# RoyiAvital/QuadraticProgramSolver

Hardware: AMD Instinct MI355X
Metric: ADMM iterations/sec (higher is better)
Workload: dtype f64

## Files before the change

quadraticprogramsolver_amd/csrc/k_loop.hip:

```cpp
#include <cstdlib>

#include "qps_kernels.h"
#include "wave_reduce.h"
#include <hip/hip_ext.h>

namespace qps {

namespace {

template <typename T> __device__ __forceinline__ T wave_sum(T v) { return wave_sum_all(v); }
__device__ __forceinline__ unsigned long long absbits(double v) { return (unsigned long long)__double_as_longlong(fabs(v)); }
__device__ __forceinline__ unsigned long long wave_max_u64(unsigned long long v) {
#pragma unroll
    for (int o = 32; o > 0; o >>= 1) { unsigned long long t = __shfl_xor(v, o, 64); v = t > v ? t : v; }
    return v;
}

template <typename T, int RB, int TRI, int THREADS>
__global__ __launch_bounds__(THREADS) void k_gemv_rows(const T* __restrict__ S, int64_t ld, const T* __restrict__ v,
                                                   T* __restrict__ out, const T* __restrict__ out0, T alpha, T beta,
                                                   int r0, int c0, int c1, BatchStride bs) {
    using V = typename VecOf<T>::type;
    if (bs.active && !bs.active[blockIdx.y]) return;
    S += (int64_t)blockIdx.y * bs.mat; v += (int64_t)blockIdx.y * bs.vin; out += (int64_t)blockIdx.y * bs.vout;
    if (out0) out0 += (int64_t)blockIdx.y * bs.vout;
    constexpr int VN = VecOf<T>::N;
    constexpr int CHUNK = THREADS * VN;
    const int tid = threadIdx.x;
    const int rb = r0 + (TRI == 1 ? (int)(gridDim.x - 1 - blockIdx.x) : (int)blockIdx.x) * RB;
    int cb = c0, ce = c1;
    if (TRI == 1) ce = min(c1, rb + RB);
    if (TRI == 2) cb = max(c0, rb);
    T acc[RB];
#pragma unroll
    for (int i = 0; i < RB; ++i) acc[i] = T(0);
    const T* Srow = S + (int64_t)rb * ld;
#pragma unroll 4
    for (int c = cb + tid * VN; c < ce; c += CHUNK) {
        const V vv = *reinterpret_cast<const V*>(v + c);
        const T* vp = reinterpret_cast<const T*>(&vv);
#pragma unroll
        for (int i = 0; i < RB; ++i) {
            typedef T NV __attribute__((ext_vector_type(VN)));
            const NV* src = reinterpret_cast<const NV*>(Srow + (int64_t)i * ld + c);
            const NV a = (TRI == 0) ? __builtin_nontemporal_load(src) : *src;
            T ap[VN];
#pragma unroll
            for (int e = 0; e < VN; ++e) ap[e] = a[e];
#pragma unroll
            for (int e = 0; e < VN; ++e) {
                bool ok = true;
                if (TRI == 1) ok = (c + e) <= (rb + i);
                if (TRI == 2) ok = (c + e) >= (rb + i);
                acc[i] += ok ? ap[e] * vp[e] : T(0);
            }
        }
    }
    __shared__ T red[THREADS / 64][RB];
#pragma unroll
    for (int i = 0; i < RB; ++i) acc[i] = wave_sum(acc[i]);
    if ((tid & 63) == 0) {
#pragma unroll
        for (int i = 0; i < RB; ++i) red[tid >> 6][i] = acc[i];
    }
    __syncthreads();
    if (tid < RB) {
        T s = T(0);
#pragma unroll
        for (int w = 0; w < THREADS / 64; ++w) s += red[w][tid];
        T r = alpha * s;
        if (beta != T(0)) r += beta * out0[rb + tid];
        out[rb + tid] = r;
    }
}

constexpr int GC_RT = 32;
template <typename T>
__global__ __launch_bounds__(256) void k_gemv_cols(const T* __restrict__ S, int64_t ld, const T* __restrict__ va,
                                                   const T* __restrict__ vb, T ca, T cb, T* __restrict__ part,
                                                   int64_t part_ld, int ncols) {
    using V = typename VecOf<T>::type;
    constexpr int VN = VecOf<T>::N;
    const int c = (blockIdx.x * 256 + threadIdx.x) * VN;
    if (c >= ncols) return;
    const int rt = blockIdx.y;
    const int rbase = rt * GC_RT;
    T acc[VN];
#pragma unroll
    for (int e = 0; e < VN; ++e) acc[e] = T(0);
    const T* Sp = S + (int64_t)rbase * ld + c;
#pragma unroll 8
    for (int i = 0; i < GC_RT; ++i) {
        T w = ca * va[rbase + i];
        if (vb) w += cb * vb[rbase + i];
        typedef T NV __attribute__((ext_vector_type(VN)));
        const NV a = __builtin_nontemporal_load(reinterpret_cast<const NV*>(Sp + (int64_t)i * ld));
#pragma unroll
        for (int e = 0; e < VN; ++e) acc[e] += a[e] * w;
    }
    V o;
    T* op = reinterpret_cast<T*>(&o);
#pragma unroll
    for (int e = 0; e < VN; ++e) op[e] = acc[e];
    *reinterpret_cast<V*>(part + (int64_t)rt * part_ld + c) = o;
}

template <typename T>
__global__ __launch_bounds__(256) void k_colsum(const T* __restrict__ part, int64_t part_ld, int ntiles,
                                                const T* __restrict__ a0, T s0, const T* __restrict__ a1, T s1,
                                                T* __restrict__ out, int ncols, BatchStride bs) {
    using V = typename VecOf<T>::type;
    constexpr int VN = VecOf<T>::N;
    if (bs.active && !bs.active[blockIdx.y]) return;
    part += (int64_t)blockIdx.y * bs.mat; out += (int64_t)blockIdx.y * bs.vout;
    if (a0) a0 += (int64_t)blockIdx.y * bs.vin;
    if (a1) a1 += (int64_t)blockIdx.y * bs.vin;
    constexpr int COLS = 128 / (int)sizeof(T);
    constexpr int CL = COLS / VN;
    constexpr int TL = 256 / CL;
    const int cl = threadIdx.x % CL, tl = threadIdx.x / CL;
    const int c = blockIdx.x * COLS + cl * VN;
    T acc[VN];
#pragma unroll
    for (int e = 0; e < VN; ++e) acc[e] = T(0);
    if (c < ncols) {
        int t = tl;
        for (; t + 7 * TL < ntiles; t += 8 * TL) {
            V v[8];
#pragma unroll
            for (int j = 0; j < 8; ++j) v[j] = *reinterpret_cast<const V*>(part + (int64_t)(t + TL * j) * part_ld + c);
#pragma unroll
            for (int j = 0; j < 8; ++j) {
                const T* vp = reinterpret_cast<const T*>(&v[j]);
#pragma unroll
                for (int e = 0; e < VN; ++e) acc[e] += vp[e];
            }
        }
        for (; t < ntiles; t += TL) {
            const V v = *reinterpret_cast<const V*>(part + (int64_t)t * part_ld + c);
            const T* vp = reinterpret_cast<const T*>(&v);
#pragma unroll
            for (int e = 0; e < VN; ++e) acc[e] += vp[e];
        }
    }
    __shared__ T red[TL][COLS + 1];
#pragma unroll
    for (int e = 0; e < VN; ++e) red[tl][cl * VN + e] = acc[e];
    __syncthreads();
    constexpr int PL = 256 / COLS;
    static_assert(TL % PL == 0 && (PL == 16 || PL == 8), "slab lanes per output");
    const int o = threadIdx.x / PL, pl = threadIdx.x % PL;
    T s = T(0);
#pragma unroll
    for (int k = 0; k < TL / PL; ++k) s += red[pl * (TL / PL) + k][o];
    s = (PL == 16) ? row16_sum_last(s) : oct_sum_all(s);
    const int oc = blockIdx.x * COLS + o;
    if (pl == PL - 1 && oc < ncols) {
        T r = s;
        if (a0) r += s0 * a0[oc];
        if (a1) r += s1 * a1[oc];
        out[oc] = r;
    }
}

template <typename T>
__global__ __launch_bounds__(256) void k_admm_update(int NP, int MP, const T* __restrict__ xx, const T* __restrict__ zz,
                                                     T* __restrict__ x, T* __restrict__ xp, T* __restrict__ z,
                                                     T* __restrict__ zp, T* __restrict__ y, const T* __restrict__ l,
                                                     const T* __restrict__ u, T alpha, T rho) {
    const int i = blockIdx.x * 256 + threadIdx.x;
    const T alpha1 = T(1) - alpha, rho1 = T(1) / rho;
    if (i < NP) {
        const T xo = x[i];
        xp[i] = xo;
        x[i] = alpha * xx[i] + alpha1 * xo;
    }
    if (i < MP) {
        const T zo = z[i], yo = y[i], zt = zz[i];
        zp[i] = zo;
        T t = alpha * zt + alpha1 * zo + rho1 * yo;
        const T lo = l[i], hi = u[i];
        const T zn = t > hi ? hi : (t < lo ? lo : t);
        z[i] = zn;
        y[i] = yo + rho * (alpha * zt + alpha1 * zo - zn);
    }
}

template <typename T>
__global__ __launch_bounds__(256) void k_check_norms(int n, int m, const T* __restrict__ Ax, const T* __restrict__ Px,
                                                     const T* __restrict__ Aty, const T* __restrict__ q,
                                                     const T* __restrict__ x, const T* __restrict__ xp,
                                                     const T* __restrict__ z, const T* __restrict__ zp,
                                                     unsigned long long* __restrict__ slots, int dual_only, BatchStride bs) {
    if (bs.active && !bs.active[blockIdx.y]) return;
    {
        const int64_t on = (int64_t)blockIdx.y * bs.vin, om = (int64_t)blockIdx.y * bs.vout;
        Ax += om; z += om; zp += om; Px += on; Aty += on; q += on; x += on; xp += on; slots += (int64_t)blockIdx.y * 16;
    }
    unsigned long long v[9];
#pragma unroll
    for (int k = 0; k < 9; ++k) v[k] = 0ull;
    for (int i = blockIdx.x * 256 + threadIdx.x; i < max(n, m); i += gridDim.x * 256) {
        if (i < m && !dual_only) {
            const double ax = (double)Ax[i], zi = (double)z[i];
            v[0] = max(v[0], absbits((double)(Ax[i] - z[i])));
            v[2] = max(v[2], absbits(ax));
            v[3] = max(v[3], absbits(zi));
            v[8] = max(v[8], absbits((double)(z[i] - zp[i])));
        }
        if (i < n) {
            v[1] = max(v[1], absbits((double)(Px[i] + q[i] + Aty[i])));
            v[4] = max(v[4], absbits((double)Px[i]));
            v[5] = max(v[5], absbits((double)Aty[i]));
            v[6] = max(v[6], absbits((double)q[i]));
            if (!dual_only) v[7] = max(v[7], absbits((double)(x[i] - xp[i])));
        }
    }
#pragma unroll
    for (int k = 0; k < 9; ++k) {
        v[k] = wave_max_u64(v[k]);
        if ((threadIdx.x & 63) == 0 && v[k] != 0ull) atomicMax(&slots[k], v[k]);
    }
}

__device__ __forceinline__ double jmax(double a, double b) { return (isnan(a) || isnan(b)) ? (double)NAN : (a > b ? a : b); }

__global__ void k_check_decide(const unsigned long long* __restrict__ slots, double* __restrict__ res, CheckScalars cs,
                               const double* __restrict__ rho_arr, const double* __restrict__ rhorho_arr,
                               const int* __restrict__ active) {
    if (threadIdx.x != 0) return;
    const int b = blockIdx.x;
    if (active && !active[b]) return;
    slots += (int64_t)b * 16; res += (int64_t)b * 8;
    if (rho_arr) { cs.rho = rho_arr[b]; cs.rhorho = rhorho_arr[b]; cs.convFlag = 1; }
    double nv[9];
    for (int k = 0; k < 9; ++k) nv[k] = __longlong_as_double((long long)slots[k]);
    const double MIN_VAL_RHO = 1e-3, MAX_VAL_RHO = 1e6;
    const double normResPrim = nv[0], normResDual = nv[1];
    const double maxNormPrim = jmax(nv[2], nv[3]);
    const double maxNormDual = jmax(jmax(nv[4], nv[5]), nv[6]);
    double rhorho = cs.rhorho;
    if (cs.adptRho) {
        const double numeratorVal = normResPrim * maxNormDual;
        const double denominatorVal = normResDual * maxNormPrim;
        const double t = cs.rho * sqrt(numeratorVal / denominatorVal);
        rhorho = t > MAX_VAL_RHO ? MAX_VAL_RHO : (t < MIN_VAL_RHO ? MIN_VAL_RHO : t);
    }
    const double epsPrim = cs.epsAbs + cs.epsRel * maxNormPrim;
    const double epsDual = cs.epsAbs + cs.epsRel * maxNormDual;
    int flag = cs.convFlag;
    if ((normResPrim < epsPrim) && (normResDual < epsDual)) flag = 3;
    if ((nv[7] <= cs.epsAdmm) && (nv[8] <= cs.epsAdmm)) flag = 2;
    res[0] = normResPrim; res[1] = normResDual; res[2] = maxNormPrim; res[3] = maxNormDual;
    res[4] = rhorho; res[5] = (double)flag; res[6] = nv[7]; res[7] = nv[8];
}

template <typename T> __global__ void k_fill(T* p, int64_t n, T v) {
    int64_t i = (int64_t)blockIdx.x * 256 + threadIdx.x;
    if (i < n) p[i] = v;
}
template <typename T> __global__ void k_convert(const double* __restrict__ s, T* __restrict__ d, int64_t n) {
    int64_t i = (int64_t)blockIdx.x * 256 + threadIdx.x;
    if (i < n) d[i] = (T)s[i];
}
template <typename T> __global__ void k_convert_back(const T* __restrict__ s, double* __restrict__ d, int64_t n) {
    int64_t i = (int64_t)blockIdx.x * 256 + threadIdx.x;
    if (i < n) d[i] = (double)s[i];
}

}

static int env_int(const char* name, int dflt) { const char* e = getenv(name); return e ? atoi(e) : dflt; }

template <typename T, int RB, int TH>
static void gemv_rows_launch(hipStream_t st, const T* S, int64_t ld, const T* v, T* out, const T* out0, T alpha, T beta, int r0,
                             int r1, int c0, int c1, int tri, BatchStride bs) {
    dim3 grid((r1 - r0 + RB - 1) / RB, bs.count);
#define QPS_GR(TRI) hipLaunchKernelGGL((k_gemv_rows<T, RB, TRI, TH>), grid, dim3(TH), 0, st, S, ld, v, out, out0, alpha, beta, r0, c0, c1, bs)
    if (tri == 0) QPS_GR(0); else if (tri == 1) QPS_GR(1); else QPS_GR(2);
#undef QPS_GR
}

template <typename T>
void gemv_rows(hipStream_t st, const T* S, int64_t ld, const T* v, T* out, const T* out0, T alpha, T beta, int r0, int r1,
               int c0, int c1, int tri, BatchStride bs) {
    if (r1 <= r0) return;
    static const int wide_th = env_int("QPS_GEMV_WIDE_THREADS", 512);
    static const int wide_rb = env_int("QPS_GEMV_WIDE_RB", 2);
    const bool wide = (c1 - c0) >= 4 * 256 * VecOf<T>::N;
    if (!wide) { gemv_rows_launch<T, 4, 256>(st, S, ld, v, out, out0, alpha, beta, r0, r1, c0, c1, tri, bs); return; }
#define QPS_W(RB, TH) gemv_rows_launch<T, RB, TH>(st, S, ld, v, out, out0, alpha, beta, r0, r1, c0, c1, tri, bs)
    if (wide_th == 512) { if (wide_rb == 4) QPS_W(4, 512); else QPS_W(VecOf<T>::N == 2 ? 2 : 4, 512); }
    else if (wide_th == 256) { if (wide_rb == 4) QPS_W(4, 256); else QPS_W(VecOf<T>::N == 2 ? 2 : 4, 256); }
    else { if (wide_rb == 4) QPS_W(4, 1024); else QPS_W(VecOf<T>::N == 2 ? 2 : 4, 1024); }
#undef QPS_W
}

int gemv_cols_tiles(int nrows) { return (nrows + GC_RT - 1) / GC_RT; }

template <typename T>
int gemv_cols_partial(hipStream_t st, const T* S, int64_t ld, const T* va, const T* vb, T ca, T cb, T* part,
                      int64_t part_ld, int nrows, int ncols) {
    constexpr int VN = VecOf<T>::N;
    const int tiles = gemv_cols_tiles(nrows);
    if (tiles == 0) return 0;
    dim3 grid((ncols + 256 * VN - 1) / (256 * VN), tiles), block(256);
    hipLaunchKernelGGL((k_gemv_cols<T>), grid, block, 0, st, S, ld, va, vb, ca, cb, part, part_ld, ncols);
    return tiles;
}

template <typename T>
void colsum(hipStream_t st, const T* part, int64_t part_ld, int ntiles, const T* a0, T s0, const T* a1, T s1, T* out,
            int ncols, BatchStride bs) {
    constexpr int cols_wg = 128 / (int)sizeof(T);
    if (g_launch_timing.start) {
        const LaunchTiming lt = g_launch_timing;
        g_launch_timing = LaunchTiming();
        hipExtLaunchKernelGGL((k_colsum<T>), dim3((ncols + cols_wg - 1) / cols_wg, bs.count), dim3(256), 0, st, lt.start, lt.stop, 0, part, part_ld, ntiles, a0, s0, a1, s1, out, ncols, bs);
        return;
    }
    hipLaunchKernelGGL((k_colsum<T>), dim3((ncols + cols_wg - 1) / cols_wg, bs.count), dim3(256), 0, st, part, part_ld, ntiles, a0, s0, a1, s1, out, ncols, bs);
}

template <typename T>
void admm_update(hipStream_t st, int NP, int MP, const T* xx, const T* zz, T* x, T* xp, T* z, T* zp, T* y, const T* l,
                 const T* u, T alpha, T rho) {
    const int N = NP > MP ? NP : MP;
    hipLaunchKernelGGL((k_admm_update<T>), dim3((N + 255) / 256), dim3(256), 0, st, NP, MP, xx, zz, x, xp, z, zp, y, l, u, alpha, rho);
}

template <typename T>
void check_convergence(hipStream_t st, int n, int m, const T* Ax, const T* Px, const T* Aty, const T* q, const T* x,
                       const T* xp, const T* z, const T* zp, unsigned long long* scratch, double* res_dev, CheckScalars cs,
                       int dual_only, BatchStride bs, const double* rho_arr, const double* rhorho_arr) {
    if (!dual_only) (void)hipMemsetAsync(scratch, 0, 16 * sizeof(unsigned long long) * bs.count, st);
    const int N = n > m ? n : m;
    int blocks = (N + 255) / 256;
    if (blocks > 1024) blocks = 1024;
    if (blocks < 1) blocks = 1;
    hipLaunchKernelGGL((k_check_norms<T>), dim3(blocks, bs.count), dim3(256), 0, st, n, m, Ax, Px, Aty, q, x, xp, z, zp, scratch, dual_only, bs);
    hipLaunchKernelGGL(k_check_decide, dim3(bs.count), dim3(64), 0, st, scratch, res_dev, cs, rho_arr, rhorho_arr, bs.active);
}

template <typename T> void fill(hipStream_t st, T* p, int64_t n, T v) {
    if (n <= 0) return;
    hipLaunchKernelGGL((k_fill<T>), dim3((unsigned)((n + 255) / 256)), dim3(256), 0, st, p, n, v);
}
template <typename T> void convert_copy(hipStream_t st, const double* src, T* dst, int64_t n) {
    if (n <= 0) return;
    hipLaunchKernelGGL((k_convert<T>), dim3((unsigned)((n + 255) / 256)), dim3(256), 0, st, src, dst, n);
}
template <typename T> void convert_back(hipStream_t st, const T* src, double* dst, int64_t n) {
    if (n <= 0) return;
    hipLaunchKernelGGL((k_convert_back<T>), dim3((unsigned)((n + 255) / 256)), dim3(256), 0, st, src, dst, n);
}

#define INST(T)                                                                                                              \
    template void gemv_rows<T>(hipStream_t, const T*, int64_t, const T*, T*, const T*, T, T, int, int, int, int, int, BatchStride); \
    template int gemv_cols_partial<T>(hipStream_t, const T*, int64_t, const T*, const T*, T, T, T*, int64_t, int, int);      \
    template void colsum<T>(hipStream_t, const T*, int64_t, int, const T*, T, const T*, T, T*, int, BatchStride);            \
    template void admm_update<T>(hipStream_t, int, int, const T*, const T*, T*, T*, T*, T*, T*, const T*, const T*, T, T);   \
    template void check_convergence<T>(hipStream_t, int, int, const T*, const T*, const T*, const T*, const T*, const T*,    \
                                       const T*, const T*, unsigned long long*, double*, CheckScalars, int, BatchStride,     \
                                       const double*, const double*);                                                        \
    template void fill<T>(hipStream_t, T*, int64_t, T);                                                                      \
    template void convert_copy<T>(hipStream_t, const double*, T*, int64_t);                                                  \
    template void convert_back<T>(hipStream_t, const T*, double*, int64_t);
INST(double)
INST(float)
#undef INST

}
```

quadraticprogramsolver_amd/csrc/qps_dense_batch.hip:

```cpp
#include <memory>

#include "dense_chol.h"
#include "qps_batch.h"
#include "qps_internal.h"
#include "qps_kernels.h"
#include "qps_polish.h"

namespace qps {
namespace {

template <typename T> struct BatchedDenseSolver : BatchSolverBase {
    StreamLease lease; DeviceOwner mem; hipStream_t st = nullptr;
    int NP = 0, MP = 0, nb = 0, slabs = 0, rpw = 0, part_tiles = 0;
    T *A = nullptr, *P = nullptr, *q = nullptr, *l = nullptr, *u = nullptr, *PI = nullptr, *AA = nullptr, *M = nullptr, *S = nullptr,
      *tmp = nullptr, *dinv = nullptr;
    T *x = nullptr, *xp = nullptr, *xres = nullptr, *z = nullptr, *y = nullptr, *xx = nullptr, *tt = nullptr, *yv = nullptr, *part = nullptr,
      *part2 = nullptr, *part_tmp = nullptr, *sw_part = nullptr, *Px = nullptr, *Aty = nullptr;
    int* fail = nullptr; int* d_active = nullptr; double *d_rho = nullptr, *d_rhorho = nullptr;
    unsigned long long* scratch = nullptr; double* res_dev = nullptr; double* res_host = nullptr; double* stage = nullptr;
    int* h_int = nullptr; double* h_dbl = nullptr;
    bool have_AA = false; double fac_sigma = -1; int fac_nb = -1; std::vector<double> fac_rho;
    char* sb_args = nullptr; void* sb_host = nullptr;
    int cat_pass = 0, cat_sweep = 0;
    static constexpr const char* kWhat = "P + sigma I + rho A'A";

    BatchedDenseSolver(int dev, int cnt, int64_t n_, int64_t m_) {
        device = dev; n = n_; m = m_; count = cnt;
        HIPC(hipSetDevice(device));
        st = prof.st = lease.acquire(device);
        NP = roundup(n, 64); MP = roundup(m, 64);
        slabs = apass_plan<T>(NP, MP, &rpw, count);
        {
            const double s = sizeof(T), c = cnt;
            cat_pass = prof.category("apass(fused A-pass, batched)", c * s * ((double)m * n + 3.0 * n + 6.0 * m));
            cat_sweep = prof.category("sweeps(fused fwd+bwd, batched, triangle read once)", c * s * ((double)n * (n + 1) / 2 + 2.0 * n));
        }
        part_tiles = gemv_cols_tiles(MP);
        const int64_t nn = (int64_t)NP * NP, c = count;
        A = mem.dalloc<T>(c * MP * NP, st); P = mem.dalloc<T>(c * nn, st); PI = mem.dalloc<T>(c * nn, st); AA = mem.dalloc<T>(c * nn, st); M = mem.dalloc<T>(c * nn, st);
        S = mem.dalloc<T>(c * nn, st); tmp = mem.dalloc<T>(c * nn, st); dinv = mem.dalloc<T>(c * (int64_t)(NP / 64) * 4096, st);
        q = mem.dalloc<T>(c * NP, st); l = mem.dalloc<T>(c * MP, st); u = mem.dalloc<T>(c * MP, st);
        x = mem.dalloc<T>(c * NP, st); xp = mem.dalloc<T>(c * NP, st); xres = mem.dalloc<T>(c * NP, st); xx = mem.dalloc<T>(c * NP, st); tt = mem.dalloc<T>(c * NP, st);
        yv = mem.dalloc<T>(c * NP, st); Px = mem.dalloc<T>(c * NP, st); Aty = mem.dalloc<T>(c * NP, st); z = mem.dalloc<T>(c * MP, st); y = mem.dalloc<T>(c * MP, st);
        int rpw1 = 0;
        const int64_t part_slabs = std::max<int64_t>(std::max<int64_t>(c * slabs, apass_plan<T>(NP, MP, &rpw1, 1)), std::max(part_tiles, 1));
        part = mem.dalloc<T>(part_slabs * NP, st); part2 = mem.dalloc<T>(c * slabs * NP, st); part_tmp = mem.dalloc<T>((int64_t)std::max(part_tiles, 1) * NP, st);
        const int sw_slabs = sweep_fused_slabs<T>(NP, count); sw_part = mem.dalloc<T>(c * std::max(sw_slabs, 1) * NP, st);
        fail = mem.dalloc<int>(count + 4, st); d_active = mem.dalloc<int>(count + 4, st); d_rho = mem.dalloc<double>(count + 4, st); d_rhorho = mem.dalloc<double>(count + 4, st);
        scratch = mem.dalloc<unsigned long long>(16 * c, st); res_dev = mem.dalloc<double>(8 * c, st);
        res_host = mem.pinned<double>(8 * c); h_int = mem.pinned<int>(count + 4); h_dbl = mem.pinned<double>(2 * (count + 4));
        stage = mem.dalloc<double>(std::max<int64_t>((int64_t)MP * NP, nn) + 64, st);
    }
    ~BatchedDenseSolver() override {
        (void)hipSetDevice(device);
        (void)hipStreamSynchronize(st);
        prof.release_events();
    }
    std::unique_ptr<FastUploader> loader;
    void put_vec(const double* h, T* d, int64_t cnt_) {
        if (cnt_ <= 0) return;
        if (!loader) loader.reset(new FastUploader(st, device));
        loader->copy(stage, h, sizeof(double) * (size_t)cnt_);
        convert_copy<T>(st, stage, d, cnt_);
    }
    void put_matrix(const double* h, int rows, int cols, T* d) {
        if (rows <= 0 || cols <= 0) return;
        if (!loader) loader.reset(new FastUploader(st, device));
        loader->copy(stage, h, sizeof(double) * (size_t)rows * cols);
        import_colmajor<T>(st, stage, rows, rows, cols, d, NP);
    }
    void finish_loading() { HIPC(hipStreamSynchronize(st)); loader.reset(); }
    void get_dual(double* zh, double* yh) override {
        HIPC(hipSetDevice(device));
        for (int b = 0; b < count && m > 0; ++b) {
            if (zh) HIPC(download_staged<T>(st, stage, z + (int64_t)b * MP, zh + (int64_t)b * m, m));
            if (yh) HIPC(download_staged<T>(st, stage, y + (int64_t)b * MP, yh + (int64_t)b * m, m));
        }
    }
    void load_problem(int b, const double* Ph, const double* Ah, const double* qh, const double* lh, const double* uh) {
        put_matrix(Ph, (int)n, (int)n, P + (int64_t)b * NP * NP);
        put_matrix(Ah, (int)m, (int)n, A + (int64_t)b * MP * NP);
        put_vec(qh, q + (int64_t)b * NP, n); put_vec(lh, l + (int64_t)b * MP, m); put_vec(uh, u + (int64_t)b * MP, m);
    }
    DenseChol<T> chol() const { return {st, (int)n, NP, MP, P, A, PI, AA, M, S, tmp, dinv, fail}; }
    void push_state(const std::vector<double>& rho, const std::vector<double>& rhorho, const std::vector<int>& active) {
        for (int b = 0; b < count; ++b) { h_dbl[b] = rho[b]; h_dbl[count + 4 + b] = rhorho[b]; h_int[b] = active[b]; }
        HIPC(hipMemcpyAsync(d_rho, h_dbl, sizeof(double) * count, hipMemcpyHostToDevice, st));
        HIPC(hipMemcpyAsync(d_rhorho, h_dbl + count + 4, sizeof(double) * count, hipMemcpyHostToDevice, st));
        HIPC(hipMemcpyAsync(d_active, h_int, sizeof(int) * count, hipMemcpyHostToDevice, st));
        HIPC(hipStreamSynchronize(st));
    }

    void refactor_changed(const std::vector<int>& changed, double sigma, const std::vector<double>& rho, const std::vector<double>& rhorho,
                          const std::vector<int>& active, std::vector<double>& tref, bool rebuild_slabs, bool push_after) {
        const double ta = now_s();
        const DenseChol<T> ch = chol();
        const bool together = (int)changed.size() * 2 >= count;
        if (together) {
            push_state(rho, rhorho, active);
            ch.form(sigma, 0.0, false, false, count, d_rho);
            ch.factor(nb, count);
            for (int b = 0; b < count; ++b) fac_rho[b] = rho[b];
        }
        for (int b : changed) {
            if (!together) { ch.at(b).form(sigma, rho[b], false, false); ch.at(b).factor(nb); fac_rho[b] = rho[b]; }
            if (rebuild_slabs) {
                T* pb_ = part + (int64_t)b * slabs * NP;
                gemv_cols_partial<T>(st, A + (int64_t)b * MP * NP, NP, z + (int64_t)b * MP, y + (int64_t)b * MP, (T)rho[b], T(-1), part_tmp, NP, MP, NP);
                colsum<T>(st, part_tmp, NP, part_tiles, nullptr, T(0), nullptr, T(0), pb_, NP);
                if (slabs > 1) HIPC(hipMemsetAsync(pb_ + NP, 0, sizeof(T) * (size_t)(slabs - 1) * NP, st));
            }
        }
        std::vector<int> all(count);
        for (int b = 0; b < count; ++b) all[b] = b;
        ch.check(kWhat, "", h_int, count, together ? &all : &changed);
        if (push_after) push_state(rho, rhorho, active);
        const double dt = (now_s() - ta) / changed.size();
        for (int b : changed) tref[b] += dt;
    }

    void solve_batch(double* xh, const qps_params& p, qps_info* infos) override {
        HIPC(hipSetDevice(device));
        const double t0 = now_s();
        if (slabs <= 0) throw QpsError(QPS_ERR_UNSUPPORTED, "batched path needs m >= 1 and n within the fused-pass limit");
        nb = pick_nb<T>(p.trsvBlock, NP);
        const DenseChol<T> ch = chol();
        const double sigma = p.sigma, alpha = p.alpha;
        const double epsAdmm = std::fmin(p.epsAbs, p.epsRel) * 1e-2;
        std::vector<double> rho(count, p.rho), rhorho(count, p.rho), resP(count, NAN), resD(count, NAN), tref(count, 0.0);
        std::vector<int> active(count, 1), conv(count, QPS_CONV_NUM_ITR), iters(count, p.numIterations), nref(count, 0);
        HIPC(hipMemsetAsync(fail, 0, sizeof(int) * count, st));
        const bool rebuild = !(p.reuseFactor && have_AA && fac_sigma == sigma);
        if ((int)fac_rho.size() != count) fac_rho.assign(count, -1.0);
        std::vector<int> todo;
        for (int b = 0; b < count; ++b)
            if (rebuild || fac_rho[b] != p.rho || fac_nb != nb) todo.push_back(b);
        if ((int)todo.size() == count) { ch.form(sigma, p.rho, rebuild, rebuild, count); ch.factor(nb, count); }
        else for (int b : todo) { ch.at(b).form(sigma, p.rho, rebuild, rebuild); ch.at(b).factor(nb); }
        ch.check(kWhat, "", h_int, count, &todo);
        have_AA = true; fac_sigma = sigma; fac_nb = nb;
        for (int b : todo) fac_rho[b] = p.rho;
        for (int b = 0; b < count; ++b) put_vec(xh + (int64_t)b * n, x + (int64_t)b * NP, n);
        loader.reset();
        HIPC(hipMemsetAsync(z, 0, sizeof(T) * (size_t)count * MP, st));
        HIPC(hipMemsetAsync(y, 0, sizeof(T) * (size_t)count * MP, st));
        push_state(rho, rhorho, active);
        const double t1 = now_s();
        BatchStride bsS; bsS.count = count; bsS.mat = (int64_t)NP * NP; bsS.vin = NP; bsS.vout = NP; bsS.active = d_active;
        BatchStride bsC; bsC.count = count; bsC.mat = (int64_t)slabs * NP; bsC.vin = NP; bsC.vout = NP; bsC.active = d_active;
        BatchStride bsK; bsK.count = count; bsK.vin = NP; bsK.vout = MP; bsK.active = d_active;
        PassBatch pb; pb.count = count; pb.slabs = slabs; pb.rho_arr = d_rho; pb.active = d_active;
        int rhs_slabs = 0, nactive = count, ii = 0;
        const int nblk = (NP + nb - 1) / nb;
        if (p.loopVariant == 0 && nblk == 1 && admm_small_batch_supported<T>(NP, MP)) {
            const size_t ab = admm_small_args_bytes(), ob = admm_small_out_bytes();
            if (!sb_host) { sb_args = mem.dalloc<char>((int64_t)(ab + ob) * count + 64, st); sb_host = mem.pinned<char>((ab + ob) * (size_t)count + 64); }
            char* args_h = static_cast<char*>(sb_host); char* outs_h = args_h + ab * count;
            char* args_d = sb_args; char* outs_d = sb_args + ab * count;
            std::vector<int> it(count, 0);
            HIPC(hipMemsetAsync(xp, 0, sizeof(T) * (size_t)count * NP, st));
            while (nactive > 0) {
                for (int b = 0; b < count; ++b)
                    admm_small_args_set(args_h, b, (int)n, (int)m, NP, MP, it[b], active[b] ? p.numIterations : it[b], p.numItrConv, p.adptRho, rho[b], rhorho[b],
                                        sigma, alpha, p.epsAbs, p.epsRel, epsAdmm, p.fctrRho);
                HIPC(hipMemcpyAsync(args_d, args_h, ab * count, hipMemcpyHostToDevice, st));
                admm_small_batch<T>(st, count, NP, MP, args_d, A, P, S, q, l, u, x, xp, z, y, outs_d);
                HIPC(hipMemcpyAsync(outs_h, outs_d, ob * count, hipMemcpyDeviceToHost, st));
                HIPC(hipStreamSynchronize(st));
                std::vector<int> changed;
                for (int b = 0; b < count; ++b) {
                    if (!active[b]) continue;
                    int last = 0, flag = QPS_CONV_NUM_ITR, need = 0; double r8[8];
                    admm_small_read(outs_h + ob * b, &last, &flag, &need, r8);
                    it[b] = last; rhorho[b] = r8[4];
                    if (!std::isnan(r8[0]) || !std::isnan(r8[1])) { resP[b] = r8[0]; resD[b] = r8[1]; }
                    if (flag != QPS_CONV_NUM_ITR) { conv[b] = flag; iters[b] = last; active[b] = 0; --nactive; }
                    else if (need && last < p.numIterations) { rho[b] = rhorho[b]; ++nref[b]; changed.push_back(b); }
                    else { iters[b] = p.numIterations; active[b] = 0; --nactive; }
                }
                if (!changed.empty()) refactor_changed(changed, sigma, rho, rhorho, active, tref, false, false);
            }
            HIPC(hipMemcpyAsync(xres, x, sizeof(T) * (size_t)count * NP, hipMemcpyDeviceToDevice, st));
        }
        for (ii = 1; ii <= p.numIterations && nactive > 0; ++ii) {
            std::vector<int> changed;
            if (p.adptRho)
                for (int b = 0; b < count; ++b)
                    if (active[b] && ((rhorho[b] * p.fctrRho < rho[b]) || (rhorho[b] > p.fctrRho * rho[b]))) {
                        rho[b] = rhorho[b]; ++nref[b]; changed.push_back(b);
                    }
            if (!changed.empty()) refactor_changed(changed, sigma, rho, rhorho, active, tref, rhs_slabs > 0, true);
            const bool check = (ii % p.numItrConv == 0);
            colsum<T>(st, part, NP, rhs_slabs, x, (T)sigma, q, T(-1), tt, NP, bsC);
            ch.sweeps(nb, tt, yv, xx, sw_part, bsS, {&prof, cat_sweep, (prof.level == 1 && ii % 50 == 13) ? 1 : 2});
            if (check) HIPC(hipMemsetAsync(scratch, 0, 16 * sizeof(unsigned long long) * count, st));
            {
                ProfLaunchScope ps(prof, cat_pass, (prof.level == 1 && !check && ii % 50 == 38) ? 1 : (check ? 3 : 2));
                apass<T>(st, check, A, NP, NP, MP, xx, x, xp, z, y, l, u, (T)alpha, T(1), part, part2, NP, scratch, pb);
            }
            std::swap(x, xp);
            rhs_slabs = slabs;
            if (check) {
                colsum<T>(st, part2, NP, slabs, nullptr, T(0), nullptr, T(0), Aty, NP, bsC);
                BatchStride bsP = bsS; bsP.mat = (int64_t)NP * NP;
                gemv_rows<T>(st, P, NP, x, Px, nullptr, T(1), T(0), 0, NP, 0, NP, 0, bsP);
                CheckScalars cs{p.epsAbs, p.epsRel, epsAdmm, 0.0, 0.0, p.adptRho, QPS_CONV_NUM_ITR};
                check_convergence<T>(st, (int)n, (int)m, (const T*)nullptr, Px, Aty, q, x, xp, z, z, scratch, res_dev, cs, 1, bsK, d_rho, d_rhorho);
                HIPC(hipMemcpyAsync(res_host, res_dev, 8 * sizeof(double) * count, hipMemcpyDeviceToHost, st));
                HIPC(hipStreamSynchronize(st));
                prof.harvest();
                for (int b = 0; b < count; ++b) {
                    if (!active[b]) continue;
                    const double* r = res_host + 8 * b;
                    resP[b] = r[0]; resD[b] = r[1]; rhorho[b] = r[4]; conv[b] = (int)r[5];
                    if (conv[b] != QPS_CONV_NUM_ITR) {
                        active[b] = 0; iters[b] = ii; --nactive;
                        HIPC(hipMemcpyAsync(xres + (int64_t)b * NP, x + (int64_t)b * NP, sizeof(T) * NP, hipMemcpyDeviceToDevice, st));
                    }
                }
                push_state(rho, rhorho, active);
            }
        }
        for (int b = 0; b < count; ++b)
            if (active[b]) HIPC(hipMemcpyAsync(xres + (int64_t)b * NP, x + (int64_t)b * NP, sizeof(T) * NP, hipMemcpyDeviceToDevice, st));
        HIPC(hipStreamSynchronize(st));
        prof.harvest();
        const double t2 = now_s();
        std::vector<PolishReport> pol(count);
        if (p.polish)
            for (int b = 0; b < count; ++b)
                polish_dense<T>(st, n, m, NP, MP, P + (int64_t)b * NP * NP, A + (int64_t)b * MP * NP, q + (int64_t)b * NP, l + (int64_t)b * MP,
                                u + (int64_t)b * MP, y + (int64_t)b * MP, xres + (int64_t)b * NP, part, p, &pol[b]);
        for (int b = 0; b < count; ++b) {
            HIPC(download_staged<T>(st, stage, xres + (int64_t)b * NP, xh + (int64_t)b * n, n));
            if (infos) {
                qps_info& in = infos[b];
                in.convFlag = conv[b]; in.iterations = iters[b]; in.numRefactor = nref[b]; in.cgIterations = 0;
                in.rhoFinal = rho[b]; in.rhoProposed = rhorho[b]; in.resPrim = resP[b]; in.resDual = resD[b];
                in.tSetup = t1 - t0; in.tLoop = t2 - t1; in.tRefactor = tref[b];
                in.polishFlag = pol[b].flag; in.polishIterations = pol[b].minresIterations; in.tPolish = pol[b].seconds;
                in.trsvBlock = nb; in.sweepVariant = chol_sweep_variant<T>(NP, nb);
                in.sweepGaveUp = 0; in.cgExplicit = 0;
            }
        }
    }
};

}

BatchSolverBase* make_dense_batch(int device, int dtype, int count, int64_t n, int64_t m, const double* P, const double* A, const double* q, const double* l,
                                  const double* u) {
    int rpw = 0;
    const int NP = roundup(n, 64), MP = roundup(m, 64);
    if (!(count > 1 && m > 0 && (dtype == QPS_F64 ? apass_plan<double>(NP, MP, &rpw, count) : apass_plan<float>(NP, MP, &rpw, count)) > 0)) return nullptr;
    auto load = [&](auto s) -> BatchSolverBase* {
        for (int64_t b = 0; b < count; ++b) s->load_problem((int)b, P + b * n * n, A + b * m * n, q + b * n, l + b * m, u + b * m);
        s->finish_loading();
        return s.release();
    };
    if (dtype == QPS_F64) return load(std::make_unique<BatchedDenseSolver<double>>(device, count, n, m));
    return load(std::make_unique<BatchedDenseSolver<float>>(device, count, n, m));
}

}
```

quadraticprogramsolver_amd/csrc/qps_kernels.h:

```cpp
#pragma once
#ifndef QPS_NT_SLABS
#define QPS_NT_SLABS 1
#endif
#include <hip/hip_runtime.h>
#include <stdint.h>

#include <atomic>
#include <thread>

namespace qps {

constexpr int kMaxDevices = 64;
int current_device();
int device_cu_count(int device);
struct PerDeviceOnce {
    std::atomic<unsigned char> state[kMaxDevices] = {};
    template <typename F> void once(int dev, F&& f) {
        if (dev < 0 || dev >= kMaxDevices) { f(); return; }
        if (state[dev].load(std::memory_order_acquire) == 2) return;
        unsigned char expect = 0;
        if (state[dev].compare_exchange_strong(expect, 1, std::memory_order_acq_rel)) { f(); state[dev].store(2, std::memory_order_release); return; }
        while (state[dev].load(std::memory_order_acquire) != 2) std::this_thread::yield();
    }
};

struct LaunchTiming { hipEvent_t start = nullptr, stop = nullptr; };
extern thread_local LaunchTiming g_launch_timing;


struct BatchStride { int count = 1; int64_t mat = 0, vin = 0, vout = 0; const int* active = nullptr; };

template <typename T> struct VecOf;
template <> struct VecOf<double> { using type = double2; static constexpr int N = 2; };
template <> struct VecOf<float>  { using type = float4;  static constexpr int N = 4; };

template <typename T>
void gemv_rows(hipStream_t st, const T* S, int64_t ld, const T* v, T* out, const T* out0, T alpha, T beta,
               int r0, int r1, int c0, int c1, int tri, BatchStride bs = BatchStride());

template <typename T>
int gemv_cols_partial(hipStream_t st, const T* S, int64_t ld, const T* va, const T* vb, T ca, T cb,
                      T* part, int64_t part_ld, int nrows, int ncols);
int gemv_cols_tiles(int nrows);

template <typename T>
void colsum(hipStream_t st, const T* part, int64_t part_ld, int ntiles, const T* a0, T s0, const T* a1, T s1,
            T* out, int ncols, BatchStride bs = BatchStride());

template <typename T>
void admm_update(hipStream_t st, int NP, int MP, const T* xx, const T* zz, T* x, T* xp, T* z, T* zp, T* y,
                 const T* l, const T* u, T alpha, T rho);

struct CheckScalars { double epsAbs, epsRel, epsAdmm, rho, rhorho; int adptRho; int convFlag; };
template <typename T>
void check_convergence(hipStream_t st, int n, int m, const T* Ax, const T* Px, const T* Aty, const T* q, const T* x,
                       const T* xp, const T* z, const T* zp, unsigned long long* scratch , double* res_dev,
                       CheckScalars cs, int dual_only = 0, BatchStride bs = BatchStride(), const double* rho_arr = nullptr,
                       const double* rhorho_arr = nullptr);

template <typename T> int apass_plan(int NP, int MP, int* rows_per_wg, int count = 1);
template <typename T> int apass_max_np();
struct PassBatch { int count = 1; int slabs = 0; const double* rho_arr = nullptr; const int* active = nullptr; int pq_me = 0; };
template <typename T>
void apass(hipStream_t st, bool check, const T* A, int64_t ld, int NP, int MP, const T* xx, const T* x_old, T* x_new, T* z,
           T* y, const T* l, const T* u, T alpha, T rho, T* part, T* part2, int64_t part_ld, unsigned long long* slots,
           PassBatch pb = PassBatch());
template <typename T> int apass_proxqp_slabs(int NP, int MP);
template <typename T>
int apass_kkt(hipStream_t st, const T* A, int64_t ld, int NP, int MP, const T* vx, const T* vlam, const T* mask, T delta, T* out_lam,
              T* part, int64_t part_ld);
template <typename T>
int apass_proxqp(hipStream_t st, const T* G, int64_t ld, int NP, int MP, int me, const T* x, T* x_scratch, T* slack, T* dual,
                 const T* g, T rho, T* part, int64_t part_ld);

template <typename T> bool sweep_fused_supported(int NP);
template <typename T> int sweep_fused_slabs(int NP, int count = 1);
template <typename T>
int sweep_fused(hipStream_t st, const T* S, int64_t ld, int NP, const T* v, T* part, int64_t part_ld, BatchStride bs = BatchStride());

template <typename T> struct PanelArgs {
    const T* Mat = nullptr; int64_t ld = 0; int rows = 0, K = 0;
    const T* B = nullptr; int npanel = 0;
    T* out = nullptr;
    const T* q = nullptr; T *x = nullptr, *xp = nullptr;
    T *z = nullptr, *zp = nullptr, *y = nullptr, *w = nullptr; const T *l = nullptr, *u = nullptr;
    const int* active = nullptr;
    T alpha = T(0), rho = T(1), sigma = T(0);
    const T *rho_row = nullptr, *rho1_row = nullptr;
};
enum class SharedPanelOp {
    product,
    rhs,
    forward,
    backward,
    backward_x,
    rows_zy,
    rows_zy_scaled,
    start_z
};
template <typename T> void shared_panel(hipStream_t st, SharedPanelOp op, const PanelArgs<T>& a);
bool shared_panel_small(int rows, int K, size_t elem);
template <typename T>
void shared_check(hipStream_t st, int n, int m, int NP, int MP, int npanel, const T* Ax, const T* Px, const T* Aty, const T* q, const T* x, const T* xp,
                  const T* z, const T* zp, unsigned long long* slots, double* res_dev, const int* active, double epsAbs, double epsRel, double epsAdmm,
                  double rho, const int* kd = nullptr, const int* ke = nullptr);
int shared_cert_blocks(int n, int m);
template <typename T>
void shared_deltas(hipStream_t st, int n, int m, int NP, int MP, int npanel, const T* x, const T* xp, const T* y, const T* yp, const T* l, const T* u,
                   const int* active, T* dx, T* dyh);
template <typename T>
void shared_certificates(hipStream_t st, int n, int m, int NP, int MP, int npanel, const T* dx, const T* dyh, const T* Adx, const T* Pdx, const T* Atdy,
                         const T* q, const T* l, const T* u, const int* active, const int* kd, const int* ke, double* part, double* res_dev, double epsP,
                         double epsD);
template <typename T> void equil_rownorm(hipStream_t st, const T* M, int rows, int K, const int* kr, const int* kc, double* out, double* lo);
void equil_update(hipStream_t st, int len, const double* a, const double* b, int* k);
template <typename T> void scale_two_sided(hipStream_t st, T* M, int rows, int cols, const int* kr, const int* kc, int sign);
template <typename T> void panel_rowscale(hipStream_t st, const T* src, const int* k, int sign, int rowsP, int npanel, T* dst);
template <typename T> void scale_entries(hipStream_t st, T* v, const int* e, int sign, int64_t cnt);
constexpr int REFRESH_VALUES_THREADS = 256;
template <typename T> void refresh_values(hipStream_t st, const double* src, const int* map, const int* e, int64_t cnt, T* dst);
constexpr int VALIDATE_VALUES_THREADS = 256;
constexpr int VALIDATE_VERDICT_KEYS = 4;
template <typename T>
void validate_values(hipStream_t st, const double* src, int64_t cnt, const int* partner, const int* cp, const int* ri, int ncols, const int* e,
                     unsigned long long* verdict);
template <typename T> struct CsrPanelMatrix { int rows = 0; const int* rp = nullptr; const int* ci = nullptr; const T* va = nullptr; int spr = 1; };
int csr_panel_spr(int64_t nnz, int rows);
template <typename T> void csr_panel(hipStream_t st, const CsrPanelMatrix<T>& M, const T* B, int rowsB, T* out, int rowsOut, int npanel);
template <typename T> void to_panels(hipStream_t st, const double* src, int count, int len, int rowsP, T* dst);
template <typename T> void from_panels(hipStream_t st, const T* src, int count, int len, int rowsP, double* dst);
template <typename T> void transpose_rowmajor(hipStream_t st, const T* src, int64_t lds, int rows, int cols, T* dst, int64_t ldd);
template <typename T> void scale_rows(hipStream_t st, const T* src, const T* scale, int rows, int cols, T* dst);
template <typename T> void panel_w(hipStream_t st, const T* z, const T* y, const int* active, const T* rho_row, T rho, int MP, int npanel, T* w);

struct SharedPolishState { double beta, oldb, dbar, epsln, phibar, cs, sn, bnorm, tol, alfa; int itn, done, flag, maxit; };
struct SharedPolishGeom { int n = 0, m = 0, rowsN = 0, rowsM = 0, npanel = 0; };
template <typename T> struct SharedPolishProducts { const T* mask = nullptr; T* wl = nullptr; const T *Ax = nullptr, *Px = nullptr, *Aty = nullptr; };
int shared_polish_blocks(int rowsN, int rowsM);
template <typename T>
void shared_polish_setup(hipStream_t st, const SharedPolishGeom& g, const T* q, const T* l, const T* u, const T* y, T* mask, T* gv, int* counts);
template <typename T> void shared_polish_wl(hipStream_t st, const SharedPolishGeom& g, const T* mask, const T* v, T* wl);
template <typename T>
void shared_polish_rhs(hipStream_t st, const SharedPolishGeom& g, const int* live, const T* gv, const T* t, const SharedPolishProducts<T>& k, T* rhs);
template <typename T>
void shared_polish_begin(hipStream_t st, const SharedPolishGeom& g, const int* live, T delta, const T* b, const T* x0, const SharedPolishProducts<T>& k, T* r1,
                         T* r2, T* w0, T* w1, double* pa, double* pb, SharedPolishState* state, double tol, int maxit);
template <typename T>
void shared_polish_step(hipStream_t st, const SharedPolishGeom& g, SharedPolishState* cur, SharedPolishState* nxt, T delta, const SharedPolishProducts<T>& k,
                        T* c, T* r1, T* r2, T* w1, const T* w2, T* x, double* pa, double* pb);
template <typename T> void shared_polish_add(hipStream_t st, const SharedPolishGeom& g, const int* live, const SharedPolishState* state, T* t, T* tt);
template <typename T> void shared_polish_select(hipStream_t st, const SharedPolishGeom& g, const int* take, const T* t, T* x);

struct CgPanelState { double res2, prev2, tol; int itn, done; };
template <typename T> struct CgPanelArgs {
    int n = 0, m = 0, npanel = 0;
    CsrPanelMatrix<T> P, A, At;
    int spr_op = 1;
    const T *q = nullptr, *lo = nullptr, *hi = nullptr; T *x = nullptr, *xp = nullptr, *z = nullptr, *zp = nullptr, *y = nullptr;
    T *xx = nullptr, *r = nullptr, *u = nullptr, *c = nullptr, *v = nullptr, *t = nullptr; const T* w = nullptr;
    double *part_uc = nullptr, *part_rr = nullptr; CgPanelState* state = nullptr;
    const int* active = nullptr;
    const T *rho_row = nullptr, *rho1_row = nullptr;
    T rho = T(1), sigma = T(0), alpha = T(0);
    const T *rho_col = nullptr, *rho1_col = nullptr;
    double eps_pcg = 0; int max_it = 0;
};
int cg_panel_op_spr(int64_t nnzP, int64_t nnzA, int n);
int cg_panel_op_blocks(int rows, int spr);
int cg_panel_vec_blocks(int rows);
template <typename T> void cg_panel_begin(hipStream_t st, const CgPanelArgs<T>& a);
template <typename T> void cg_panel_iteration(hipStream_t st, const CgPanelArgs<T>& a, int cur, bool first);
template <typename T> void cg_panel_finish(hipStream_t st, const CgPanelArgs<T>& a, int cur);
template <typename T> void cg_panel_post(hipStream_t st, const CgPanelArgs<T>& a);
template <typename T> void cg_panel_w(hipStream_t st, const CgPanelArgs<T>& a, T* w);

template <typename T> bool admm_small_supported(int n, int m, int NP, int MP);
template <typename T> void transpose_small(hipStream_t st, const T* A, int NP, int MP, T* At);
template <typename T> bool admm_small_batch_supported(int NP, int MP);
size_t admm_small_args_bytes();
void admm_small_args_set(void* host_array, int idx, int n, int m, int NP, int MP, int it_begin, int it_end, int numItrConv, int adptRho, double rho,
                         double rhorho, double sigma, double alpha, double epsAbs, double epsRel, double epsAdmm, double fctrRho);
template <typename T>
void admm_small_batch(hipStream_t st, int count, int NP, int MP, const void* args_dev, const T* A, const T* P, const T* S, const T* q, const T* l,
                      const T* u, T* x, T* xp, T* z, T* y, void* outs_dev);
template <typename T>
void admm_small(hipStream_t st, int n, int m, int NP, int MP, int it_begin, int it_end, int numItrConv, int adptRho, double rho,
                double rhorho, double sigma, double alpha, double epsAbs, double epsRel, double epsAdmm, double fctrRho, const T* A,
                const T* At, const T* P, const T* S, const T* q, const T* l, const T* u, T* x, T* xp, T* z, T* y, void* out_dev);
size_t admm_small_out_bytes();
void admm_small_read(const void* host_copy, int* last_it, int* convFlag, int* need_rho, double* res8);

template <typename T> void fill(hipStream_t st, T* p, int64_t n, T v);
template <typename T> void convert_copy(hipStream_t st, const double* src, T* dst, int64_t n);
template <typename T> void convert_back(hipStream_t st, const T* src, double* dst, int64_t n);
template <typename T> inline hipError_t upload_staged(hipStream_t st, double* stage, const double* h, T* d, int64_t n) {
    if (n <= 0) return hipSuccess;
    const hipError_t e = hipMemcpyAsync(stage, h, sizeof(double) * (size_t)n, hipMemcpyHostToDevice, st);
    if (e != hipSuccess) return e;
    convert_copy<T>(st, stage, d, n);
    return hipStreamSynchronize(st);
}
template <typename T> inline hipError_t download_staged(hipStream_t st, double* stage, const T* d, double* h, int64_t n) {
    if (n <= 0) return hipSuccess;
    convert_back<T>(st, d, stage, n);
    const hipError_t e = hipMemcpyAsync(h, stage, sizeof(double) * (size_t)n, hipMemcpyDeviceToHost, st);
    return e != hipSuccess ? e : hipStreamSynchronize(st);
}

template <typename T>
void import_colmajor(hipStream_t st, const double* src, int64_t lds, int rows, int cols, T* dst, int64_t ldd);

template <typename T>
void gemm(hipStream_t st, int M, int N, int K, T alpha, const T* A, int64_t lda, bool a_kcontig, const T* B, int64_t ldb,
          bool b_kcontig, T beta, T* C, int64_t ldc, bool lower_only, int batch = 1, int64_t sA = 0, int64_t sB = 0,
          int64_t sC = 0, int ktri = 0);

template <typename T> void assemble_M(hipStream_t st, int NP, const T* PI, const T* AA, T rho, T* M, int batch = 1,
                                      const double* rho_arr = nullptr);
template <typename T> void make_PI(hipStream_t st, int n, int NP, const T* P, T sigma, T* PI, int batch = 1);

inline int64_t chol_scratch_elems(int NP) { return (int64_t)((NP / 64 + 1) / 2) * 3 * 4096 + 64; }
inline bool chol_scratch_fits(int NP) { return chol_scratch_elems(NP) <= (int64_t)NP * NP; }
template <typename T> void cholesky(hipStream_t st, int NP, T* M, T* dinv, int* fail_dev, int batch = 1, T* scratch = nullptr);

template <typename T> void build_sweep_matrix(hipStream_t st, int NP, int nb, const T* L, const T* dinv, T* S, T* tmp, int batch = 1, bool premul = false);

template <typename T> bool trsv_blocked_supported(int NP, int nb);
template <typename T> int64_t trsv_blocked_pub_words(int NP);
struct TrsvBlockedPair { int dev; hipStream_t stream; TrsvBlockedPair(int device, hipStream_t st); ~TrsvBlockedPair(); TrsvBlockedPair(const TrsvBlockedPair&) = delete; };
void trsv_blocked_forget_stream(int device, hipStream_t st);
template <typename T>
void trsv_blocked(hipStream_t st, bool bwd, const T* S, int64_t ld, int NP, int nb, const T* v, T* out, unsigned long long* pub,
                  unsigned epoch, unsigned* abort_word, int mode = 0);

}
```

Before: 14650.

## Batch per-problem vector uploads/downloads into single strided convert kernels

Per-problem loops of staged copies (each with its own conversion kernel and stream sync) for x, z, y and the final solution are replaced by one bulk host-device copy plus one strided convert kernel per vector. The per-problem device-to-device copies into xres become a single masked hold kernel that runs only when polishing needs it. push_state is skipped when rho, rhorho and active are unchanged. This cuts launch and sync overhead per batch but adds extra device staging memory and selection logic.

```diff
diff --git a/quadraticprogramsolver_amd/csrc/k_loop.hip b/quadraticprogramsolver_amd/csrc/k_loop.hip
--- a/quadraticprogramsolver_amd/csrc/k_loop.hip
+++ b/quadraticprogramsolver_amd/csrc/k_loop.hip
@@ -267,6 +267,25 @@
     int64_t i = (int64_t)blockIdx.x * 256 + threadIdx.x;
     if (i < n) d[i] = (double)s[i];
 }
+template <typename T> __global__ void k_convert_rows(const double* __restrict__ s, T* __restrict__ d, int len, int64_t ld, int64_t total) {
+    const int64_t k = (int64_t)blockIdx.x * 256 + threadIdx.x;
+    if (k >= total) return;
+    const int64_t b = k / len;
+    d[b * ld + (k - b * len)] = (T)s[k];
+}
+template <typename T>
+__global__ void k_convert_rows_back(const T* __restrict__ cur, const T* __restrict__ held, const int* __restrict__ sel, double* __restrict__ d, int len, int64_t ld,
+                                    int64_t total) {
+    const int64_t k = (int64_t)blockIdx.x * 256 + threadIdx.x;
+    if (k >= total) return;
+    const int64_t b = k / len;
+    const T* s = (!sel || sel[b]) ? cur : held;
+    d[k] = (double)s[b * ld + (k - b * len)];
+}
+template <typename T> __global__ void k_hold_rows(const T* __restrict__ cur, T* __restrict__ held, const int* __restrict__ sel, int64_t ld, int64_t total) {
+    const int64_t k = (int64_t)blockIdx.x * 256 + threadIdx.x;
+    if (k < total && sel[k / ld]) held[k] = cur[k];
+}
 
 }
 
@@ -354,6 +373,21 @@
     if (n <= 0) return;
     hipLaunchKernelGGL((k_convert_back<T>), dim3((unsigned)((n + 255) / 256)), dim3(256), 0, st, src, dst, n);
 }
+template <typename T> void convert_rows(hipStream_t st, const double* src, int count, int len, T* dst, int64_t ld) {
+    const int64_t total = (int64_t)count * len;
+    if (total <= 0) return;
+    hipLaunchKernelGGL((k_convert_rows<T>), dim3((unsigned)((total + 255) / 256)), dim3(256), 0, st, src, dst, len, ld, total);
+}
+template <typename T> void convert_rows_back(hipStream_t st, const T* cur, const T* held, const int* sel, int count, int len, int64_t ld, double* dst) {
+    const int64_t total = (int64_t)count * len;
+    if (total <= 0) return;
+    hipLaunchKernelGGL((k_convert_rows_back<T>), dim3((unsigned)((total + 255) / 256)), dim3(256), 0, st, cur, held, sel, dst, len, ld, total);
+}
+template <typename T> void hold_rows(hipStream_t st, const T* cur, T* held, const int* sel, int count, int64_t ld) {
+    const int64_t total = (int64_t)count * ld;
+    if (total <= 0) return;
+    hipLaunchKernelGGL((k_hold_rows<T>), dim3((unsigned)((total + 255) / 256)), dim3(256), 0, st, cur, held, sel, ld, total);
+}
 
 #define INST(T)                                                                                                              \
     template void gemv_rows<T>(hipStream_t, const T*, int64_t, const T*, T*, const T*, T, T, int, int, int, int, int, BatchStride); \
@@ -365,7 +399,10 @@
                                        const double*, const double*);                                                        \
     template void fill<T>(hipStream_t, T*, int64_t, T);                                                                      \
     template void convert_copy<T>(hipStream_t, const double*, T*, int64_t);                                                  \
-    template void convert_back<T>(hipStream_t, const T*, double*, int64_t);
+    template void convert_back<T>(hipStream_t, const T*, double*, int64_t);                                                  \
+    template void convert_rows<T>(hipStream_t, const double*, int, int, T*, int64_t);                                        \
+    template void convert_rows_back<T>(hipStream_t, const T*, const T*, const int*, int, int, int64_t, double*);             \
+    template void hold_rows<T>(hipStream_t, const T*, T*, const int*, int, int64_t);
 INST(double)
 INST(float)
 #undef INST
diff --git a/quadraticprogramsolver_amd/csrc/qps_dense_batch.hip b/quadraticprogramsolver_amd/csrc/qps_dense_batch.hip
--- a/quadraticprogramsolver_amd/csrc/qps_dense_batch.hip
+++ b/quadraticprogramsolver_amd/csrc/qps_dense_batch.hip
@@ -17,7 +17,7 @@
     T *x = nullptr, *xp = nullptr, *xres = nullptr, *z = nullptr, *y = nullptr, *xx = nullptr, *tt = nullptr, *yv = nullptr, *part = nullptr,
       *part2 = nullptr, *part_tmp = nullptr, *sw_part = nullptr, *Px = nullptr, *Aty = nullptr;
     int* fail = nullptr; int* d_active = nullptr; double *d_rho = nullptr, *d_rhorho = nullptr;
-    unsigned long long* scratch = nullptr; double* res_dev = nullptr; double* res_host = nullptr; double* stage = nullptr;
+    unsigned long long* scratch = nullptr; double* res_dev = nullptr; double* res_host = nullptr; double* stage = nullptr; double* vstage = nullptr;
     int* h_int = nullptr; double* h_dbl = nullptr;
     bool have_AA = false; double fac_sigma = -1; int fac_nb = -1; std::vector<double> fac_rho;
     char* sb_args = nullptr; void* sb_host = nullptr;
@@ -50,6 +50,7 @@
         scratch = mem.dalloc<unsigned long long>(16 * c, st); res_dev = mem.dalloc<double>(8 * c, st);
         res_host = mem.pinned<double>(8 * c); h_int = mem.pinned<int>(count + 4); h_dbl = mem.pinned<double>(2 * (count + 4));
         stage = mem.dalloc<double>(std::max<int64_t>((int64_t)MP * NP, nn) + 64, st);
+        vstage = mem.dalloc<double>(c * std::max<int64_t>(n, m), st);
     }
     ~BatchedDenseSolver() override {
         (void)hipSetDevice(device);
@@ -70,12 +71,22 @@
         import_colmajor<T>(st, stage, rows, rows, cols, d, NP);
     }
     void finish_loading() { HIPC(hipStreamSynchronize(st)); loader.reset(); }
+    void put_rows(const double* h, int len, T* d, int64_t ld) {
+        if (len <= 0) return;
+        if (!loader) loader.reset(new FastUploader(st, device));
+        loader->copy(vstage, h, sizeof(double) * (size_t)count * (size_t)len);
+        convert_rows<T>(st, vstage, count, len, d, ld);
+    }
+    void get_rows(const T* cur, const T* held, const int* sel, int len, int64_t ld, double* h) {
+        if (len <= 0) return;
+        convert_rows_back<T>(st, cur, held, sel, count, len, ld, vstage);
+        HIPC(hipMemcpyAsync(h, vstage, sizeof(double) * (size_t)count * (size_t)len, hipMemcpyDeviceToHost, st));
+        HIPC(hipStreamSynchronize(st));
+    }
     void get_dual(double* zh, double* yh) override {
         HIPC(hipSetDevice(device));
-        for (int b = 0; b < count && m > 0; ++b) {
-            if (zh) HIPC(download_staged<T>(st, stage, z + (int64_t)b * MP, zh + (int64_t)b * m, m));
-            if (yh) HIPC(download_staged<T>(st, stage, y + (int64_t)b * MP, yh + (int64_t)b * m, m));
-        }
+        if (zh) get_rows(z, z, nullptr, (int)m, MP, zh);
+        if (yh) get_rows(y, y, nullptr, (int)m, MP, yh);
     }
     void load_problem(int b, const double* Ph, const double* Ah, const double* qh, const double* lh, const double* uh) {
         put_matrix(Ph, (int)n, (int)n, P + (int64_t)b * NP * NP);
@@ -83,12 +94,16 @@
         put_vec(qh, q + (int64_t)b * NP, n); put_vec(lh, l + (int64_t)b * MP, m); put_vec(uh, u + (int64_t)b * MP, m);
     }
     DenseChol<T> chol() const { return {st, (int)n, NP, MP, P, A, PI, AA, M, S, tmp, dinv, fail}; }
+    std::vector<double> pushed_rho, pushed_rhorho; std::vector<int> pushed_active; bool pushed = false, rhorho_read = true;
     void push_state(const std::vector<double>& rho, const std::vector<double>& rhorho, const std::vector<int>& active) {
+        if (pushed && rho == pushed_rho && active == pushed_active && (!rhorho_read || rhorho == pushed_rhorho)) return;
+        pushed = false;
         for (int b = 0; b < count; ++b) { h_dbl[b] = rho[b]; h_dbl[count + 4 + b] = rhorho[b]; h_int[b] = active[b]; }
         HIPC(hipMemcpyAsync(d_rho, h_dbl, sizeof(double) * count, hipMemcpyHostToDevice, st));
         HIPC(hipMemcpyAsync(d_rhorho, h_dbl + count + 4, sizeof(double) * count, hipMemcpyHostToDevice, st));
         HIPC(hipMemcpyAsync(d_active, h_int, sizeof(int) * count, hipMemcpyHostToDevice, st));
         HIPC(hipStreamSynchronize(st));
+        pushed_rho = rho; pushed_rhorho = rhorho; pushed_active = active; pushed = true;
     }
 
     void refactor_changed(const std::vector<int>& changed, double sigma, const std::vector<double>& rho, const std::vector<double>& rhorho,
@@ -140,8 +155,9 @@
         ch.check(kWhat, "", h_int, count, &todo);
         have_AA = true; fac_sigma = sigma; fac_nb = nb;
         for (int b : todo) fac_rho[b] = p.rho;
-        for (int b = 0; b < count; ++b) put_vec(xh + (int64_t)b * n, x + (int64_t)b * NP, n);
+        put_rows(xh, (int)n, x, NP);
         loader.reset();
+        rhorho_read = !p.adptRho;
         HIPC(hipMemsetAsync(z, 0, sizeof(T) * (size_t)count * MP, st));
         HIPC(hipMemsetAsync(y, 0, sizeof(T) * (size_t)count * MP, st));
         push_state(rho, rhorho, active);
@@ -151,6 +167,7 @@
         BatchStride bsK; bsK.count = count; bsK.vin = NP; bsK.vout = MP; bsK.active = d_active;
         PassBatch pb; pb.count = count; pb.slabs = slabs; pb.rho_arr = d_rho; pb.active = d_active;
         int rhs_slabs = 0, nactive = count, ii = 0;
+        bool all_in_xres = false;
         const int nblk = (NP + nb - 1) / nb;
         if (p.loopVariant == 0 && nblk == 1 && admm_small_batch_supported<T>(NP, MP)) {
             const size_t ab = admm_small_args_bytes(), ob = admm_small_out_bytes();
@@ -181,6 +198,7 @@
                 if (!changed.empty()) refactor_changed(changed, sigma, rho, rhorho, active, tref, false, false);
             }
             HIPC(hipMemcpyAsync(xres, x, sizeof(T) * (size_t)count * NP, hipMemcpyDeviceToDevice, st));
+            all_in_xres = true;
         }
         for (ii = 1; ii <= p.numIterations && nactive > 0; ++ii) {
             std::vector<int> changed;
@@ -221,8 +239,7 @@
                 push_state(rho, rhorho, active);
             }
         }
-        for (int b = 0; b < count; ++b)
-            if (active[b]) HIPC(hipMemcpyAsync(xres + (int64_t)b * NP, x + (int64_t)b * NP, sizeof(T) * NP, hipMemcpyDeviceToDevice, st));
+        if (p.polish && !all_in_xres) { hold_rows<T>(st, x, xres, d_active, count, NP); all_in_xres = true; }
         HIPC(hipStreamSynchronize(st));
         prof.harvest();
         const double t2 = now_s();
@@ -231,17 +248,15 @@
             for (int b = 0; b < count; ++b)
                 polish_dense<T>(st, n, m, NP, MP, P + (int64_t)b * NP * NP, A + (int64_t)b * MP * NP, q + (int64_t)b * NP, l + (int64_t)b * MP,
                                 u + (int64_t)b * MP, y + (int64_t)b * MP, xres + (int64_t)b * NP, part, p, &pol[b]);
-        for (int b = 0; b < count; ++b) {
-            HIPC(download_staged<T>(st, stage, xres + (int64_t)b * NP, xh + (int64_t)b * n, n));
-            if (infos) {
-                qps_info& in = infos[b];
-                in.convFlag = conv[b]; in.iterations = iters[b]; in.numRefactor = nref[b]; in.cgIterations = 0;
-                in.rhoFinal = rho[b]; in.rhoProposed = rhorho[b]; in.resPrim = resP[b]; in.resDual = resD[b];
-                in.tSetup = t1 - t0; in.tLoop = t2 - t1; in.tRefactor = tref[b];
-                in.polishFlag = pol[b].flag; in.polishIterations = pol[b].minresIterations; in.tPolish = pol[b].seconds;
-                in.trsvBlock = nb; in.sweepVariant = chol_sweep_variant<T>(NP, nb);
-                in.sweepGaveUp = 0; in.cgExplicit = 0;
-            }
+        get_rows(all_in_xres ? xres : x, xres, all_in_xres ? nullptr : d_active, (int)n, NP, xh);
+        for (int b = 0; b < count && infos; ++b) {
+            qps_info& in = infos[b];
+            in.convFlag = conv[b]; in.iterations = iters[b]; in.numRefactor = nref[b]; in.cgIterations = 0;
+            in.rhoFinal = rho[b]; in.rhoProposed = rhorho[b]; in.resPrim = resP[b]; in.resDual = resD[b];
+            in.tSetup = t1 - t0; in.tLoop = t2 - t1; in.tRefactor = tref[b];
+            in.polishFlag = pol[b].flag; in.polishIterations = pol[b].minresIterations; in.tPolish = pol[b].seconds;
+            in.trsvBlock = nb; in.sweepVariant = chol_sweep_variant<T>(NP, nb);
+            in.sweepGaveUp = 0; in.cgExplicit = 0;
         }
     }
 };
diff --git a/quadraticprogramsolver_amd/csrc/qps_kernels.h b/quadraticprogramsolver_amd/csrc/qps_kernels.h
--- a/quadraticprogramsolver_amd/csrc/qps_kernels.h
+++ b/quadraticprogramsolver_amd/csrc/qps_kernels.h
@@ -193,6 +193,9 @@
 template <typename T> void fill(hipStream_t st, T* p, int64_t n, T v);
 template <typename T> void convert_copy(hipStream_t st, const double* src, T* dst, int64_t n);
 template <typename T> void convert_back(hipStream_t st, const T* src, double* dst, int64_t n);
+template <typename T> void convert_rows(hipStream_t st, const double* src, int count, int len, T* dst, int64_t ld);
+template <typename T> void convert_rows_back(hipStream_t st, const T* cur, const T* held, const int* sel, int count, int len, int64_t ld, double* dst);
+template <typename T> void hold_rows(hipStream_t st, const T* cur, T* held, const int* sel, int count, int64_t ld);
 template <typename T> inline hipError_t upload_staged(hipStream_t st, double* stage, const double* h, T* d, int64_t n) {
     if (n <= 0) return hipSuccess;
     const hipError_t e = hipMemcpyAsync(stage, h, sizeof(double) * (size_t)n, hipMemcpyHostToDevice, st);
```

New measurement: 14530. Within noise of the previous version (-0.8%).
